# acoustic-warfare/beamforming-lk

Hardware: NVIDIA B200
Metric: power_maps_per_sec (higher is better)
Workload: dtype f32

## Files before the change

### beamforming-lk_b200/bflk/__init__.py

```python
import ctypes as C
import os

import numpy as np

_PKG = os.path.dirname(os.path.dirname(os.path.abspath(__file__)))
LIB_PATH = os.path.join(_PKG, "libbflk.so")

N_SAMPLES = 256
WINDOW = 1024
ELEMENTS = 64
SAMPLE_RATE = 48828.0
PROPAGATION_SPEED = 340.0

KERNEL_AUTO, KERNEL_GENERIC, KERNEL_TILED, KERNEL_BCAST, KERNEL_TILED_FMA2 = 0, 1, 2, 3, 4

SYMBOLS = [
    "bflk_default_config", "bflk_version", "bflk_create", "bflk_destroy", "bflk_last_error",
    "bflk_set_geometry", "bflk_set_tiled_geometry", "bflk_get_geometry", "bflk_set_channel_mask",
    "bflk_set_grid_fov", "bflk_set_grid_tables", "bflk_set_grid_shape", "bflk_set_direction_range", "bflk_get_n_directions",
    "bflk_get_grid", "bflk_get_tables", "bflk_steer_tables", "bflk_power_map", "bflk_power_map_i32",
    "bflk_power_map_batch", "bflk_power_map_batch_submit", "bflk_power_map_batch_wait", "bflk_power_map_batch_i32", "bflk_power_map_batch_i32_dev",
    "bflk_power_map_batch_dev", "bflk_power_map_batch_dev_submit", "bflk_power_map_batch_dev_join", "bflk_set_kernel", "bflk_set_channel_split", "bflk_launch_shape", "bflk_get_kernel", "bflk_launch_count", "bflk_enable_timing",
    "bflk_kernel_time_ms", "bflk_fp32_peak_tflops", "bflk_set_window", "bflk_set_window_dev", "bflk_miso", "bflk_miso_dev", "bflk_monopulse", "bflk_set_fir",
    "bflk_pin_host", "bflk_unpin_host", "bflk_heatmap", "bflk_resize_u8", "bflk_targets", "bflk_calibrate", "bflk_ingest_i32",
    "bflk_stream_open", "bflk_stream_close", "bflk_stream_push", "bflk_stream_push_i32", "bflk_stream_power_maps",
    "bflk_stream_discard", "bflk_stream_status", "bflk_stream_window",
    "bflk_comm_unique_id", "bflk_comm_init_rank", "bflk_comm_info", "bflk_shard_plan",
    "bflk_power_map_batch_sharded_dev", "bflk_power_map_batch_sharded_dev_submit", "bflk_power_map_batch_sharded_dev_join", "bflk_power_map_batch_sharded", "bflk_power_map_batch_sharded_submit", "bflk_power_map_batch_sharded_wait",
    "bflk_group_create", "bflk_group_destroy", "bflk_group_size", "bflk_group_handle", "bflk_group_last_error",
    "bflk_group_set_geometry", "bflk_group_set_tiled_geometry", "bflk_group_set_channel_mask", "bflk_group_set_grid_fov",
    "bflk_group_set_kernel", "bflk_group_power_map_batch", "bflk_group_power_map_batch_dev", "bflk_group_synchronize",
]


class Config(C.Structure):
    _fields_ = [("n_channels", C.c_int32), ("frame_len", C.c_int32), ("history", C.c_int32),
                ("window_len", C.c_int32), ("sample_rate", C.c_double), ("propagation_speed", C.c_double),
                ("device", C.c_int32), ("reserved", C.c_int32)]


class Target(C.Structure):
    _fields_ = [("theta", C.c_double), ("phi", C.c_double), ("power", C.c_float), ("probability", C.c_float),
                ("direction", C.c_int32), ("row", C.c_int32), ("col", C.c_int32), ("reserved", C.c_int32)]


# ... 27 lines not shown
    L.bflk_get_geometry.argtypes = [vp, vp]
    L.bflk_set_channel_mask.argtypes = [vp, vp, i32]
    L.bflk_set_grid_fov.argtypes = [vp, i32, i32, f32]
    L.bflk_set_grid_tables.argtypes = [vp, vp, vp, i32]
    L.bflk_set_grid_shape.argtypes = [vp, i32, i32]
    L.bflk_set_direction_range.argtypes = [vp, i32, i32]
    L.bflk_get_n_directions.argtypes = [vp, C.POINTER(i32), C.POINTER(i32), C.POINTER(i32)]
    L.bflk_get_grid.argtypes = [vp, vp, vp]
    L.bflk_get_tables.argtypes = [vp, vp, vp]
    L.bflk_steer_tables.argtypes = [vp, vp, vp, i32, vp, vp]
    L.bflk_power_map.argtypes = [vp, vp, vp]
    L.bflk_power_map_i32.argtypes = [vp, vp, vp]
    L.bflk_power_map_batch.argtypes = [vp, vp, i64, i32, vp]
    L.bflk_power_map_batch_submit.argtypes = [vp, vp, i64, i32, vp]
    L.bflk_power_map_batch_wait.argtypes = [vp]
    L.bflk_power_map_batch_i32.argtypes = [vp, vp, i64, i32, vp]
    L.bflk_power_map_batch_i32_dev.argtypes = [vp, vp, i64, i32, vp, vp]
    L.bflk_power_map_batch_dev.argtypes = [vp, vp, i64, i32, vp, vp]
    L.bflk_power_map_batch_dev_submit.argtypes = [vp, vp, i64, i32, vp, vp]
    L.bflk_power_map_batch_dev_join.argtypes = [vp, vp]
    L.bflk_set_kernel.argtypes = [vp, i32]
    L.bflk_set_channel_split.argtypes = [vp, i32]
    L.bflk_launch_shape.argtypes = [i32, i32, i32, i32, i32, i32, i32, C.POINTER(i32), C.POINTER(i32)]
    L.bflk_launch_count.argtypes = [vp]
    L.bflk_launch_count.restype = i64
    L.bflk_get_kernel.argtypes = [vp, C.POINTER(i32), C.POINTER(i32), C.POINTER(i32)]
    L.bflk_enable_timing.argtypes = [vp, i32]
    L.bflk_kernel_time_ms.argtypes = [vp, C.POINTER(f32), C.POINTER(i32), C.POINTER(f32), C.POINTER(i32)]
    L.bflk_fp32_peak_tflops.argtypes = [vp, C.POINTER(f32)]
    L.bflk_set_window.argtypes = [vp, vp]
    L.bflk_set_window_dev.argtypes = [vp, vp]
    L.bflk_miso.argtypes = [vp, vp, vp, i32, vp, vp, vp]
    L.bflk_miso_dev.argtypes = [vp, vp, vp, i32, vp, vp, vp, vp]
    L.bflk_monopulse.argtypes = [vp, vp, vp, i32, C.c_double, C.c_double, C.c_double, vp, vp, vp, vp, vp, vp]
    L.bflk_set_fir.argtypes = [vp, vp, i32, i32]
    L.bflk_heatmap.argtypes = [vp, vp, i32, vp, C.POINTER(i32), C.POINTER(f32)]
    L.bflk_pin_host.argtypes = [vp, C.c_size_t]
    L.bflk_unpin_host.argtypes = [vp]
    L.bflk_resize_u8.argtypes = [vp, vp, i32, i32, i32, i32, vp]
    L.bflk_targets.argtypes = [vp, vp, i32, f32, vp, C.POINTER(i32)]
    L.bflk_calibrate.argtypes = [vp, vp, i32, f32, vp, vp, C.POINTER(i32), C.POINTER(f32), C.POINTER(f32)]
    L.bflk_ingest_i32.argtypes = [vp, vp, i32, i32, vp]
    L.bflk_stream_open.argtypes = [vp, i32]
    L.bflk_stream_close.argtypes = [vp]
    L.bflk_stream_push.argtypes = [vp, vp, i32]
    L.bflk_stream_push_i32.argtypes = [vp, vp, i32]
# ... 37 lines not shown

def _ptr(a):
    return a.ctypes.data_as(C.c_void_p)


def shard_plan(n_directions, n_frames, n_ranks, rank, dir_groups=0):
    L = load_library()
    a, b, c, d = C.c_int32(), C.c_int32(), C.c_int32(), C.c_int32()
    rc = L.bflk_shard_plan(n_directions, n_frames, n_ranks, dir_groups, rank, C.byref(a), C.byref(b), C.byref(c), C.byref(d))
    if rc != 0:
        raise BflkError(rc, f"bflk_shard_plan({n_directions}, {n_frames}, {n_ranks}, {dir_groups}, {rank})")
    return a.value, b.value, c.value, d.value


def launch_shape(rows, cols, n_channels, n_frames=1, frame_len=256, n_sms=148, channel_split=False):
    L = load_library()
    w, s = C.c_int32(), C.c_int32()
    rc = L.bflk_launch_shape(rows, cols, n_channels, frame_len, n_frames, n_sms, 1 if channel_split else 0, C.byref(w), C.byref(s))
    if rc != 0:
        raise BflkError(rc, f"bflk_launch_shape({rows}, {cols}, {n_channels}, {frame_len}, {n_frames}, {n_sms})")
    return w.value, s.value


def comm_unique_id():
    L = load_library()
    buf = (C.c_uint8 * 128)()
    rc = L.bflk_comm_unique_id(buf)
    if rc != 0:
        raise BflkError(rc, "bflk_comm_unique_id: NCCL is not available")
    return bytes(buf)


def tile_origins(nx, ny, pitch=0.16):
    o = [[(i - (nx - 1) / 2) * pitch, (j - (ny - 1) / 2) * pitch, 0.0] for j in range(ny) for i in range(nx)]
    return np.asarray(o, np.float32)


class Beamformer:

    def __init__(self, n_channels=ELEMENTS, frame_len=N_SAMPLES, history=N_SAMPLES, window_len=WINDOW,
                 sample_rate=SAMPLE_RATE, propagation_speed=PROPAGATION_SPEED, device=0):
        self._L = load_library()
        cfg = Config()
        self._L.bflk_default_config(C.byref(cfg))
        cfg.n_channels, cfg.frame_len, cfg.history, cfg.window_len = n_channels, frame_len, history, window_len
        cfg.sample_rate, cfg.propagation_speed, cfg.device = sample_rate, propagation_speed, device
# ... 405 lines not shown
```

### beamforming-lk_b200/csrc/bflk_api.cu

```cuda
#include <algorithm>
#include <cmath>
#include <cstdlib>
#include <cstring>
#include <functional>
#include <memory>

#include "bflk_internal.h"

using namespace bflk;

static thread_local std::string g_create_error;

static int create_fail(int code, const std::string &msg) {
    g_create_error = msg;
    return code;
}

bflk_handle::~bflk_handle() {
    for (const Stream *s : {&stream, &copy_stream, &lane[0], &lane[1]}) s->sync();
    comm_release(this);
}

extern "C" {

// ... 26 lines not shown
    if (e != cudaSuccess || n_dev <= 0)
        return create_fail(BFLK_ERR_NO_DEVICE, std::string("bflk_create: no CUDA device (") + cudaGetErrorString(e) +
                                                   "); this library has no CPU fallback");
    if (cfg->device < 0 || cfg->device >= n_dev) return create_fail(BFLK_ERR_INVALID, "bflk_create: device ordinal out of range");
    cudaDeviceProp prop;
    if ((e = cudaGetDeviceProperties(&prop, cfg->device)) != cudaSuccess)
        return create_fail(BFLK_ERR_CUDA, std::string("cudaGetDeviceProperties: ") + cudaGetErrorString(e));
    if (prop.major != 10)
        return create_fail(BFLK_ERR_NO_DEVICE, "bflk_create: device is not sm_100 (kernels are built for sm_100a only)");
    if ((e = cudaSetDevice(cfg->device)) != cudaSuccess)
        return create_fail(BFLK_ERR_CUDA, std::string("cudaSetDevice: ") + cudaGetErrorString(e));
    cudaGetLastError();
    std::unique_ptr<bflk_handle> h(new bflk_handle());
    if ((e = cudaGetLastError()) != cudaSuccess)
        return create_fail(BFLK_ERR_CUDA, std::string("bflk_create: cannot create the streams and events: ") + cudaGetErrorString(e));
    h->cfg = *cfg;
    h->sm_count = prop.multiProcessorCount;
    auto env_int = [](const char *name, int dflt) { const char *v = getenv(name); return v && *v ? atoi(v) : dflt; };
    h->tuning.tile_nch = env_int("BFLK_TILE_NCH", 0);
    h->tuning.tile_warps = env_int("BFLK_TILE_WARPS", 0);
    h->tuning.tile_stages = env_int("BFLK_TILE_STAGES", 0);
    h->tuning.tile_pairs = env_int("BFLK_TILE_PAIRS", 0);
    h->tuning.tile_mode = env_int("BFLK_TILE_MODE", -1);
    h->tuning.no_ksplit = env_int("BFLK_NO_KSPLIT", 0);
    h->tuning.lat_warps = env_int("BFLK_LAT_WARPS", 0);
    h->tuning.lat_split = env_int("BFLK_LAT_SPLIT", 0);
    h->tuning.chunk_mib = env_int("BFLK_CHUNK_MIB", 0);
    *out = h.release();
    return BFLK_OK;
}

int bflk_destroy(bflk_handle *h) {
    if (!h) return BFLK_ERR_INVALID;
    cudaSetDevice(h->cfg.device);
    delete h;
    return BFLK_OK;
}

static void invalidate_tables(bflk_handle *h) {
    h->have_grid = false;
    h->tiles_valid = false;
    h->bcast_valid = false;
    h->n_dir = 0;
    h->dir_first = h->dir_count = 0;
    h->last_map_on_device = false;
}

int bflk_set_geometry(bflk_handle *h, const float *xyz, int32_t n_channels) {
    if (!h) return BFLK_ERR_INVALID;
    if (!xyz || n_channels != h->cfg.n_channels)
        return h->fail(BFLK_ERR_INVALID, "bflk_set_geometry: expected %d channels, got %d", h->cfg.n_channels, n_channels);
    BFLK_CUDA(h, cudaSetDevice(h->cfg.device));
    h->xyz.assign(xyz, xyz + 3 * (size_t)n_channels);
    BFLK_CUDA(h, h->d_xyz.reserve(3 * (size_t)n_channels));
    BFLK_CUDA(h, cudaMemcpyAsync(h->d_xyz.p, h->xyz.data(), h->xyz.size() * sizeof(float), cudaMemcpyHostToDevice, h->stream));
    BFLK_CUDA(h, cudaStreamSynchronize(h->stream));
    h->have_geometry = true;
    invalidate_tables(h);
    if (h->index.empty()) return bflk_set_channel_mask(h, nullptr, 0);
    return BFLK_OK;
}

int bflk_set_tiled_geometry(bflk_handle *h, int32_t n_tiles, const float *origins) {
    if (!h) return BFLK_ERR_INVALID;
// ... 22 lines not shown
    return BFLK_OK;
}

int bflk_set_channel_mask(bflk_handle *h, const int32_t *index, int32_t usable) {
    if (!h) return BFLK_ERR_INVALID;
    const int C = h->cfg.n_channels;
    std::vector<int32_t> idx;
    if (!index) {
        idx.resize(C);
        for (int c = 0; c < C; c++) idx[c] = c;
    } else {
        if (usable <= 0 || usable > C) return h->fail(BFLK_ERR_INVALID, "bflk_set_channel_mask: usable=%d out of range", usable);
        idx.assign(index, index + usable);
        for (int v : idx)
            if (v < 0 || v >= C) return h->fail(BFLK_ERR_INVALID, "bflk_set_channel_mask: channel %d out of range", v);
    }
    BFLK_CUDA(h, cudaSetDevice(h->cfg.device));
    h->index = idx;
    h->bcast_valid = false;
    BFLK_CUDA(h, h->d_index.reserve(idx.size()));
    BFLK_CUDA(h, cudaMemcpyAsync(h->d_index.p, h->index.data(), idx.size() * sizeof(int32_t), cudaMemcpyHostToDevice, h->stream));
    BFLK_CUDA(h, cudaStreamSynchronize(h->stream));
    h->tiles_valid = false;
    return BFLK_OK;
}

static DirTrig make_trig(double theta, double phi) {
    const float az = static_cast<float>(phi);
    const float ay = -static_cast<float>(theta);
    DirTrig t;
    t.cz = static_cast<float>(std::cos((double)az));
    t.sz = static_cast<float>(std::sin((double)az));
    t.cy = static_cast<float>(std::cos((double)ay));
    t.sy = static_cast<float>(std::sin((double)ay));
    return t;
}

static float delay_scale(const bflk_handle *h) { return (float)(h->cfg.sample_rate / h->cfg.propagation_speed); }

static int run_steer_tables(bflk_handle *h, const double *theta, const double *phi, int n, int32_t *d_off, float *d_frac,
                            int32_t *max_delay) {
    BFLK_CUDA(h, h->p_trig.reserve(n));
    BFLK_CUDA(h, h->d_trig.reserve(n));
    BFLK_CUDA(h, h->d_misc.reserve(4));
    BFLK_CUDA(h, h->p_misc.reserve(4));
    for (int i = 0; i < n; i++) h->p_trig.p[i] = make_trig(theta[i], phi[i]);
// ... 86 lines not shown
    if (min_off < 0 || max_off > h->cfg.history)
        return h->fail(BFLK_ERR_RANGE, "bflk_set_grid_tables: offsets must lie in [0, history = %d]; got [%d, %d]",
                       h->cfg.history, min_off, max_off);
    const int max_delay = h->cfg.history - min_off;
    h->theta.clear();
    h->phi.clear();
    h->rows = h->cols = 0;
    h->n_dir = n_directions;
    h->dir_first = 0;
    h->dir_count = n_directions;
    h->max_delay = max_delay;
    h->have_grid = true;
    return BFLK_OK;
}

int bflk_set_grid_shape(bflk_handle *h, int32_t rows, int32_t cols) {
    if (!h) return BFLK_ERR_INVALID;
    if (!h->have_grid) return h->fail(BFLK_ERR_STATE, "bflk_set_grid_shape: set the tables first");
    if (rows <= 0 || cols <= 0 || (int64_t)rows * cols != h->n_dir)
        return h->fail(BFLK_ERR_INVALID, "bflk_set_grid_shape: %d x %d is not the %d directions of the tables", rows, cols, h->n_dir);
    h->rows = rows;
    h->cols = cols;
    h->tiles_valid = false;
    h->bcast_valid = false;
    return BFLK_OK;
}

int bflk_set_direction_range(bflk_handle *h, int32_t first, int32_t count) {
    if (!h) return BFLK_ERR_INVALID;
    if (!h->have_grid) return h->fail(BFLK_ERR_STATE, "bflk_set_direction_range: set the grid first");
    if (first < 0 || count <= 0 || first + count > h->n_dir)
        return h->fail(BFLK_ERR_INVALID, "bflk_set_direction_range: [%d, %d) outside grid of %d", first, first + count, h->n_dir);
    h->dir_first = first;
    h->dir_count = count;
    h->tiles_valid = false;
    h->bcast_valid = false;
    h->last_map_on_device = false;
    return BFLK_OK;
}

int bflk_get_n_directions(const bflk_handle *h, int32_t *total, int32_t *first, int32_t *count) {
    if (!h || !h->have_grid) return BFLK_ERR_STATE;
    if (total) *total = h->n_dir;
    if (first) *first = h->dir_first;
    if (count) *count = h->dir_count;
    return BFLK_OK;
}

int bflk_get_grid(const bflk_handle *h, double *theta, double *phi) {
    if (!h || !h->have_grid || h->theta.empty()) return BFLK_ERR_STATE;
    if (theta) std::memcpy(theta, h->theta.data(), h->theta.size() * sizeof(double));
    if (phi) std::memcpy(phi, h->phi.data(), h->phi.size() * sizeof(double));
    return BFLK_OK;
}

int bflk_get_tables(const bflk_handle *hc, int32_t *offsets, float *fractions) {
    bflk_handle *h = const_cast<bflk_handle *>(hc);
    if (!h) return BFLK_ERR_INVALID;
// ... 121 lines not shown
    if (pack_launches) *pack_launches = n[1];
    return BFLK_OK;
}

}

namespace bflk {

int64_t min_stream_samples(const bflk_handle *h, int n_frames) {
    return (int64_t)(n_frames - 1) * h->cfg.frame_len + h->cfg.history + h->cfg.frame_len + 1;
}

int ensure_tiles(bflk_handle *h, int fast, int want_warps) {
    if (h->tiles_valid && h->tiles_fast == fast && h->tiles_want_warps == want_warps) return BFLK_OK;
    BFLK_CUDA(h, cudaEventSynchronize(h->caller_event));
    h->tiles_valid = false;
    h->tiles_fast = fast;
    h->tiles_want_warps = want_warps;
    h->tiles_usable = false;
    if (h->rows <= 0 || h->cols <= 0) {
        h->tiles_valid = true;
        return BFLK_OK;
    }
    const int cols = h->cols;
    const int row0 = (h->dir_first / cols) & ~1;
    const int row1 = (h->dir_first + h->dir_count - 1) / cols;
    const int tile_rows = (row1 - row0) / 2 + 1, tile_cols = (cols + 1) / 2;
    const int n_tiles = tile_rows * tile_cols;
    const int usable = (int)h->index.size();
    BFLK_CUDA(h, h->d_tile_dirs.reserve((size_t)n_tiles * 4));
    BFLK_CUDA(h, h->d_misc.reserve(4));
    BFLK_CUDA(h, h->p_misc.reserve(4));
    const int stage_off = das_tile_geometry(h->cfg.history, h->max_delay, 0).stage_off;
    BFLK_CUDA(h, cudaMemsetAsync(h->d_misc.p, 0, 4 * sizeof(int32_t), h->stream));
    for (int mode = 0; mode < 3; mode++) {
        BFLK_CUDA(h, launch_build_tiles(h->d_off.p, h->d_frac.p, h->cfg.n_channels, h->d_index.p, usable, h->rows, cols,
                                        h->dir_first, h->dir_count, stage_off, 0, 1, mode, -1, 0, nullptr, nullptr, n_tiles,
                                        h->d_misc.p, h->stream));
        h->launches++;
    }
    BFLK_CUDA(h, cudaMemcpyAsync(h->p_misc.p, h->d_misc.p, 3 * sizeof(int32_t), cudaMemcpyDeviceToHost, h->stream));
    BFLK_CUDA(h, cudaStreamSynchronize(h->stream));
    const int span0 = h->p_misc.p[0], span1 = h->p_misc.p[1], span2 = h->p_misc.p[2];
    int mode = 0;
    const int pair_span = std::min(span1, span2), pair_mode = span1 <= span2 ? 1 : 2;
    if (span0 > 3 && pair_span <= 3) mode = pair_mode;
    else if (span0 > 7 && pair_span <= 5) mode = pair_mode;
    const int forced = h->tuning.tile_mode;
    if (forced == 0 || ((forced == 1 || forced == 2) && h->p_misc.p[forced] <= 5)) mode = forced;
    h->n_tiles = n_tiles;
    h->tile_smax = h->p_misc.p[mode];
    h->tile_geom = das_tile_geometry(h->cfg.history, h->max_delay, h->tile_smax, n_tiles, mode, fast, &h->tuning, want_warps);
    h->tiles_usable = h->tile_smax <= das_tile_max_span() && h->cfg.frame_len >= 256 && h->cfg.frame_len % 2 == 0 &&
                      h->tile_geom.stages >= 3;
    if (!h->tiles_usable) {
        h->tiles_valid = true;
        return BFLK_OK;
    }
    const size_t entries = tile_table_entries(n_tiles, usable, h->tile_geom.warps);
    const size_t ent_bytes = das_tile_entry_bytes(h->tile_geom);
    BFLK_CUDA(h, h->d_tiles.reserve(entries * ent_bytes));
    BFLK_CUDA(h, cudaMemsetAsync(h->d_tiles.p, 0, entries * ent_bytes, h->stream));
    BFLK_CUDA(h, launch_build_tiles(h->d_off.p, h->d_frac.p, h->cfg.n_channels, h->d_index.p, usable, h->rows, cols,
                                    h->dir_first, h->dir_count, stage_off, h->tile_geom.copy_bytes, h->tile_geom.warps, mode,
                                    2 * h->tile_geom.nch - 9, fast, h->d_tiles.p,
                                    h->d_tile_dirs.p, n_tiles, h->d_misc.p, h->stream));
    h->launches++;
    BFLK_CUDA(h, cudaStreamSynchronize(h->stream));
    h->tiles_valid = true;
    return BFLK_OK;
}

}

extern "C" {

static int ensure_bcast(bflk_handle *h) {
    if (h->bcast_valid) return BFLK_OK;
    BFLK_CUDA(h, cudaEventSynchronize(h->caller_event));
    const int first = h->dir_first, count = h->dir_count;
    std::vector<int32_t> globals;
    if (h->rows > 0 && h->cols > 0) {
        float minx = 1e30f, maxx = -1e30f, miny = 1e30f, maxy = -1e30f;
        for (size_t c = 0; c < h->xyz.size() / 3; c++) {
            minx = std::min(minx, h->xyz[3 * c]); maxx = std::max(maxx, h->xyz[3 * c]);
            miny = std::min(miny, h->xyz[3 * c + 1]); maxy = std::max(maxy, h->xyz[3 * c + 1]);
        }
        const int TR = (maxx - minx >= maxy - miny) ? 8 : 4, TC = 32 / TR;
// ... 1093 lines not shown
```

### beamforming-lk_b200/csrc/bflk_internal.h

```cpp
#pragma once

#include <cuda_runtime.h>

#include <cstdarg>
#include <algorithm>
#include <cstdint>
#include <cstdio>
#include <memory>
#include <string>
#include <vector>

#include "../../include/bflk.h"

namespace bflk {

struct DirTrig {
    float cz, sz;
    float cy, sy;
};

struct __align__(16) TileEntry {
    uint32_t win_off;
    uint32_t deltas;
    int32_t span;
// ... 10 lines not shown
    float comp[4];
};

struct __align__(16) TileEntryFastDual {
    uint32_t cls_a[4], cls_b[4];
    float frac[4], comp[4];
    uint32_t deltas;
    int32_t span;
    int32_t reserved[2];
};

constexpr int kTileCC = 8;
inline size_t tile_table_entries(int n_tiles, int usable, int warps) {
    const size_t groups = (n_tiles + warps - 1) / warps, stages = (usable + kTileCC - 1) / kTileCC;
    return groups * stages * warps * kTileCC;
}

struct Tuning {
    int tile_nch = 0;
    int tile_warps = 0;
    int tile_stages = 0;
    int tile_pairs = 0;
    int tile_mode = -1;
    int lat_warps = 0;
    int lat_split = 0;
    int no_ksplit = 0;
    int chunk_mib = 0;
};

struct TileGeometry {
    int stage_off = 0;
    int nch = 0;
    int warps = 0;
    int tmpl_warps = 0;
    int fast = 0;
    int mode = 0;
    int row_chunks = 0;
    int copy_bytes = 0;
    int row_bytes = 0;
    int stages = 0;
    int pairs_per_cta = 0;
    int ksplit = 1;
};

constexpr int kBcastCC = 8;
struct BcastEntry {
// ... 93 lines not shown
    bool have_geometry = false;
    std::vector<float> xyz;
    std::vector<int32_t> index;
    bflk::DevBuf<float> d_xyz;
    bflk::DevBuf<int32_t> d_index;

    bool have_grid = false;
    int32_t rows = 0, cols = 0;
    int32_t n_dir = 0;
    int32_t dir_first = 0, dir_count = 0;
    int32_t max_delay = 0;
    std::vector<double> theta, phi;
    bflk::DevBuf<int32_t> d_off;
    bflk::DevBuf<float> d_frac;

    bool tiles_valid = false;
    bool tiles_usable = false;
    int tiles_fast = 0;
    int tiles_want_warps = 0;
    int32_t n_tiles = 0;
    int32_t tile_smax = 0;
    bflk::DevBuf<char> d_tiles;
    bflk::DevBuf<int32_t> d_tile_dirs;
    bflk::TileGeometry tile_geom;

    bool bcast_valid = false;
    int32_t bcast_tiles = 0;
    bflk::BcastGeometry bcast_geom;
    bflk::DevBuf<bflk::BcastEntry> d_bcast_table;
    bflk::DevBuf<int32_t> d_bcast_dirs;
    bflk::DevBuf<int32_t> d_bcast_globals;

    bflk::DevBuf<float> d_fir;
    int32_t fir_phases = 0, fir_taps = 0;

    const float *resident_window = nullptr;
    int64_t resident_stride = 0;
    std::unique_ptr<bflk::Session> session;
    bflk::DevBuf<int32_t> d_wire;
    bflk::DevBuf<uint8_t> d_bytes;
    bflk::DevBuf<float> d_async_in[2], d_async_out[2];
    bflk::Event async_done[2];
    uint64_t async_seq = 0;
    int async_pending = 0;
    bflk::DevBuf<float> d_maps;
    bool last_map_on_device = false;
// ... 40 lines not shown
        char buf[512];
        va_list ap;
        va_start(ap, fmt);
        vsnprintf(buf, sizeof(buf), fmt, ap);
        va_end(ap);
        error = buf;
        return code;
    }
};

#define BFLK_CUDA(h, expr)                                                                              \
    do {                                                                                                \
        cudaError_t _e = (expr);                                                                        \
        if (_e != cudaSuccess)                                                                          \
            return (h)->fail(BFLK_ERR_CUDA, "%s failed: %s (%s:%d)", #expr, cudaGetErrorString(_e), __FILE__, __LINE__); \
    } while (0)

namespace bflk {

cudaError_t launch_steer_tables(const DirTrig *d_trig, int n_dir, const float *d_xyz, int C, float k_scale,
                                int history, int32_t *d_off, float *d_frac, int32_t *d_maxdelay, cudaStream_t st);
cudaError_t launch_offset_range(const int32_t *d_off, size_t n, int32_t *d_maxoff, int32_t *d_minoff, cudaStream_t st);
cudaError_t launch_build_tiles(const int32_t *d_off, const float *d_frac, int C, const int32_t *d_index, int usable,
                               int rows, int cols, int first, int count, int stage_off, int copy_bytes, int warps,
                               int mode, int pair_span, int fast, void *d_tiles, int32_t *d_tile_dirs, int n_tiles,
                               int32_t *d_maxspan, cudaStream_t st);

struct GenericArgs {
    const float *stream;
    int64_t row_stride;
    int n_frames;
    int frame_len;
    int frame_stride;
    const int32_t *off;
    const float *frac;
    int C;
    const int32_t *index;
    int usable;
    int n_dir;
    float *power;
    float *audio;
    float norm;
    const float *fir = nullptr;
    int fir_phases = 0, fir_taps = 0;
};
cudaError_t launch_das_generic(const GenericArgs &a, cudaStream_t st);

constexpr int kMisoInline = 128;
struct MisoArgs {
// ... 114 lines not shown
```

### beamforming-lk_b200/csrc/tables.cu

```cuda
#include "bflk_internal.h"
#include "steer.cuh"

namespace bflk {

__global__ void __launch_bounds__(128) steer_tables_kernel(const DirTrig *__restrict__ trig, const float *__restrict__ xyz,
                                                           int C, float k_scale, int history, int32_t *__restrict__ off,
                                                           float *__restrict__ frac, int32_t *__restrict__ maxdelay) {
    extern __shared__ float s_del[];
    __shared__ float s_red[4];
    const int d = blockIdx.x;
    const DirTrig t = trig[d];
    float mn = INFINITY;
    for (int c = threadIdx.x; c < C; c += blockDim.x) {
        float z = steer_z(t, xyz[3 * c + 0], xyz[3 * c + 1], xyz[3 * c + 2]);
        float del = __fmul_rn(z, k_scale);
        s_del[c] = del;
        mn = fminf(mn, del);
    }
    for (int o = 16; o > 0; o >>= 1) mn = fminf(mn, __shfl_xor_sync(0xffffffffu, mn, o));
    if ((threadIdx.x & 31) == 0) s_red[threadIdx.x >> 5] = mn;
    __syncthreads();
    mn = fminf(fminf(s_red[0], s_red[1]), fminf(s_red[2], s_red[3]));
    int local_max = 0;
    for (int c = threadIdx.x; c < C; c += blockDim.x) {
// ... 22 lines not shown
        int o = off[i];
        mx = max(mx, o);
        mo = min(mo, o);
    }
    for (int o = 16; o > 0; o >>= 1) {
        mx = max(mx, __shfl_xor_sync(0xffffffffu, mx, o));
        mo = min(mo, __shfl_xor_sync(0xffffffffu, mo, o));
    }
    if ((threadIdx.x & 31) == 0) {
        atomicMax(maxoff, mx);
        atomicMin(minoff, mo);
    }
}

cudaError_t launch_offset_range(const int32_t *d_off, size_t n, int32_t *d_maxoff, int32_t *d_minoff, cudaStream_t st) {
    int blocks = (int)((n + 255) / 256);
    if (blocks > 1184) blocks = 1184;
    if (blocks < 1) blocks = 1;
    max_delay_kernel<<<blocks, 256, 0, st>>>(d_off, n, d_maxoff, d_minoff);
    return cudaGetLastError();
}

__global__ void build_tiles_kernel(const int32_t *__restrict__ off, const float *__restrict__ frac, int C,
                                   const int32_t *__restrict__ index, int usable, int rows, int cols, int first,
                                   int count, int stage_off, int copy_bytes, int warps, int mode, int pair_span,
                                   int fast, void *__restrict__ tiles_raw,
                                   int32_t *__restrict__ tile_dirs, int n_tiles, int tile_cols, int row0,
                                   int32_t *__restrict__ maxspan) {
    const int t = blockIdx.x;
    if (t >= n_tiles) return;
    TileEntry *tiles = fast ? nullptr : static_cast<TileEntry *>(tiles_raw);
    TileEntryFast *tiles_fast = fast && mode == 0 ? static_cast<TileEntryFast *>(tiles_raw) : nullptr;
    TileEntryFastDual *tiles_fast2 = fast && mode != 0 ? static_cast<TileEntryFastDual *>(tiles_raw) : nullptr;
    const int tr = t / tile_cols, tc = t % tile_cols;
    int dirs[4];
#pragma unroll
    for (int slot = 0; slot < 4; slot++) {
        const int q = mode == 1 ? ((slot & 1) << 1 | (slot >> 1)) : slot;
        int r = row0 + 2 * tr + (q >> 1), c = 2 * tc + (q & 1);
        dirs[slot] = (r < rows && c < cols) ? r * cols + c : -1;
    }
    int ref = dirs[0];
#pragma unroll
    for (int slot = 1; slot < 4; slot++)
        if (ref < 0) ref = dirs[slot];
    if (threadIdx.x < 4 && tile_dirs) {
        int g = dirs[threadIdx.x];
        tile_dirs[4 * t + threadIdx.x] = (g >= first && g < first + count) ? g - first : -1;
    }
    int span_max = 0;
    for (int s = threadIdx.x; s < usable; s += blockDim.x) {
        const int c = index[s];
        int o[4];
        TileEntry e;
#pragma unroll
        for (int slot = 0; slot < 4; slot++) {
            int g = dirs[slot] >= 0 ? dirs[slot] : ref;
            o[slot] = off[(size_t)g * C + c];
            e.frac[slot] = frac[(size_t)g * C + c];
        }
        unsigned packed = 0, need_last = 0;
        int span = 0;
        if (mode == 0) {
            const int base = min(min(o[0], o[1]), min(o[2], o[3]));
// ... 57 lines not shown
            for (int w = 0; w < 2; w++) {
                const unsigned wo = (e.win_off >> (16 * w)) & 0xffffu, r = (packed >> (24 + 2 * w)) & 3;
#pragma unroll
                for (int k = 0; k < 4; k++)
                    (w ? q.cls_b : q.cls_a)[k] = (unsigned)(s % kTileCC) * 2u * (unsigned)copy_bytes + wo + ((k > 0 && r >= (unsigned)(4 - k)) ? 16u : 0u);
            }
            q.deltas = (packed & 0x10ffffffu) | need_last;
            q.span = span;
            q.reserved[0] = q.reserved[1] = 0;
#pragma unroll
            for (int k = 0; k < 4; k++) {
                q.frac[k] = e.frac[k];
                q.comp[k] = __fsub_rn(1.0f, e.frac[k]);
            }
            tiles_fast2[slot] = q;
        }
        span_max = max(span_max, span);
    }
    for (int o = 16; o > 0; o >>= 1) span_max = max(span_max, __shfl_xor_sync(0xffffffffu, span_max, o));
    if ((threadIdx.x & 31) == 0) atomicMax(maxspan + mode, span_max);
}

cudaError_t launch_build_tiles(const int32_t *d_off, const float *d_frac, int C, const int32_t *d_index, int usable,
                               int rows, int cols, int first, int count, int stage_off, int copy_bytes, int warps,
                               int mode, int pair_span, int fast, void *d_tiles, int32_t *d_tile_dirs, int n_tiles,
                               int32_t *d_maxspan, cudaStream_t st) {
    const int row0 = (first / cols) & ~1;
    const int tile_cols = (cols + 1) / 2;
    build_tiles_kernel<<<n_tiles, 128, 0, st>>>(d_off, d_frac, C, d_index, usable, rows, cols, first, count, stage_off,
                                                copy_bytes, warps, mode, pair_span, fast, d_tiles, d_tile_dirs, n_tiles, tile_cols, row0, d_maxspan);
    return cudaGetLastError();
}

}
```

### include/bflk.h

```cpp
#ifndef BFLK_H
#define BFLK_H

#include <stddef.h>
#include <stdint.h>

#ifdef __cplusplus
extern "C" {
#endif

#define BFLK_VERSION 1

typedef enum bflk_status {
    BFLK_OK = 0,
    BFLK_ERR_INVALID = -1,
    BFLK_ERR_STATE = -2,
    BFLK_ERR_CUDA = -3,
    BFLK_ERR_NO_DEVICE = -4,
    BFLK_ERR_RANGE = -5
} bflk_status;

typedef struct bflk_config {
    int32_t n_channels;
    int32_t frame_len;
    int32_t history;
// ... 25 lines not shown
int bflk_get_n_directions(const bflk_handle *h, int32_t *total, int32_t *first, int32_t *count);
int bflk_get_grid(const bflk_handle *h, double *theta, double *phi);
int bflk_get_tables(const bflk_handle *h, int32_t *offsets, float *fractions);
int bflk_steer_tables(bflk_handle *h, const double *theta, const double *phi, int32_t n_targets,
                      int32_t *offsets, float *fractions);

int bflk_power_map(bflk_handle *h, const float *window, float *power_out);
int bflk_power_map_batch(bflk_handle *h, const float *stream, int64_t n_samples, int32_t n_frames, float *power_out);
int bflk_power_map_batch_submit(bflk_handle *h, const float *stream, int64_t n_samples, int32_t n_frames, float *power_out);
int bflk_power_map_batch_wait(bflk_handle *h);
int bflk_power_map_i32(bflk_handle *h, const int32_t *frames, float *power_out);
int bflk_power_map_batch_i32(bflk_handle *h, const int32_t *frames, int64_t n_samples, int32_t n_frames, float *power_out);
int bflk_power_map_batch_i32_dev(bflk_handle *h, const int32_t *frames_dev, int64_t n_samples, int32_t n_frames,
                                 float *power_dev, void *cuda_stream);
int bflk_power_map_batch_dev(bflk_handle *h, const float *stream_dev, int64_t n_samples, int32_t n_frames,
                             float *power_dev, void *cuda_stream);
int bflk_power_map_batch_dev_submit(bflk_handle *h, const float *stream_dev, int64_t n_samples, int32_t n_frames,
                                    float *power_dev, void *cuda_stream);
int bflk_power_map_batch_dev_join(bflk_handle *h, void *cuda_stream);
int bflk_set_kernel(bflk_handle *h, int32_t which);
int bflk_set_channel_split(bflk_handle *h, int32_t on);
int bflk_launch_shape(int32_t rows, int32_t cols, int32_t n_channels, int32_t frame_len, int32_t n_frames, int32_t n_sms,
                      int32_t channel_split, int32_t *warps, int32_t *split);
int bflk_get_kernel(const bflk_handle *h, int32_t *last_used, int32_t *tile_span, int32_t *window_chunks);
int64_t bflk_launch_count(const bflk_handle *h);
int bflk_enable_timing(bflk_handle *h, int32_t on);
int bflk_fp32_peak_tflops(bflk_handle *h, float *tflops);
int bflk_kernel_time_ms(bflk_handle *h, float *das_ms, int32_t *das_launches, float *pack_ms, int32_t *pack_launches);

int bflk_stream_open(bflk_handle *h, int32_t max_frames);
int bflk_stream_close(bflk_handle *h);
int bflk_stream_push(bflk_handle *h, const float *samples, int32_t n);
int bflk_stream_push_i32(bflk_handle *h, const int32_t *rows, int32_t n);
int bflk_stream_power_maps(bflk_handle *h, int32_t max_frames, float *power_out, int64_t *first_frame, int32_t *n_frames);
int bflk_stream_discard(bflk_handle *h, int32_t keep);
int bflk_stream_status(const bflk_handle *h, int64_t *pushed, int64_t *next_frame, int32_t *ready, int64_t *skipped);
int bflk_stream_window(bflk_handle *h, int64_t frame);

int bflk_comm_unique_id(uint8_t *id128);
int bflk_comm_init_rank(bflk_handle *h, const uint8_t *id128, int32_t n_ranks, int32_t rank, int32_t dir_groups);
int bflk_comm_info(const bflk_handle *h, int32_t *n_ranks, int32_t *rank, int32_t *dir_groups, int32_t *frame_groups,
                   int64_t *collectives);
int bflk_shard_plan(int32_t n_directions, int32_t n_frames, int32_t n_ranks, int32_t dir_groups, int32_t rank,
                    int32_t *dir_first, int32_t *dir_count, int32_t *frame_first, int32_t *frame_count);
int bflk_power_map_batch_sharded_dev(bflk_handle *h, const float *stream_dev, int64_t n_samples, int32_t n_frames,
                                     float *power_all_dev, void *cuda_stream);
// ... 58 lines not shown
```

Measured before the change: 77730.

## Group tiled-kernel directions by delay similarity via matching instead of fixed 2x2 grid

Replaces the fixed 2x2 grid assignment of directions to tiles with a host-side grouping. The grouping pairs directions by delay-offset similarity using greedy-plus-augmenting matching, then pairs those pairs into tiles and refines them with local swaps. Tiles are sorted by window cost and passed to the tile builder as an explicit direction list. The aim is to cut the number of channels whose delay spread exceeds the shared window, lowering per-tile sample loads in the dual (mode != 0) tiled kernel. The grouping adds host-side setup cost, and a new error path triggers if a grouped pair's spread exceeds the window.

```diff
diff --git a/beamforming-lk_b200/bflk/__init__.py b/beamforming-lk_b200/bflk/__init__.py
--- a/beamforming-lk_b200/bflk/__init__.py
+++ b/beamforming-lk_b200/bflk/__init__.py
@@ -20,7 +20,7 @@
     "bflk_set_grid_fov", "bflk_set_grid_tables", "bflk_set_grid_shape", "bflk_set_direction_range", "bflk_get_n_directions",
     "bflk_get_grid", "bflk_get_tables", "bflk_steer_tables", "bflk_power_map", "bflk_power_map_i32",
     "bflk_power_map_batch", "bflk_power_map_batch_submit", "bflk_power_map_batch_wait", "bflk_power_map_batch_i32", "bflk_power_map_batch_i32_dev",
-    "bflk_power_map_batch_dev", "bflk_power_map_batch_dev_submit", "bflk_power_map_batch_dev_join", "bflk_set_kernel", "bflk_set_channel_split", "bflk_launch_shape", "bflk_get_kernel", "bflk_launch_count", "bflk_enable_timing",
+    "bflk_power_map_batch_dev", "bflk_power_map_batch_dev_submit", "bflk_power_map_batch_dev_join", "bflk_set_kernel", "bflk_set_channel_split", "bflk_launch_shape", "bflk_tile_grouping", "bflk_get_kernel", "bflk_launch_count", "bflk_enable_timing",
     "bflk_kernel_time_ms", "bflk_fp32_peak_tflops", "bflk_set_window", "bflk_set_window_dev", "bflk_miso", "bflk_miso_dev", "bflk_monopulse", "bflk_set_fir",
     "bflk_pin_host", "bflk_unpin_host", "bflk_heatmap", "bflk_resize_u8", "bflk_targets", "bflk_calibrate", "bflk_ingest_i32",
     "bflk_stream_open", "bflk_stream_close", "bflk_stream_push", "bflk_stream_push_i32", "bflk_stream_power_maps",
@@ -94,6 +94,7 @@
     L.bflk_set_kernel.argtypes = [vp, i32]
     L.bflk_set_channel_split.argtypes = [vp, i32]
     L.bflk_launch_shape.argtypes = [i32, i32, i32, i32, i32, i32, i32, C.POINTER(i32), C.POINTER(i32)]
+    L.bflk_tile_grouping.argtypes = [vp, i32, i32, i32, i32, i32, vp, C.POINTER(i32), C.POINTER(i64)]
     L.bflk_launch_count.argtypes = [vp]
     L.bflk_launch_count.restype = i64
     L.bflk_get_kernel.argtypes = [vp, C.POINTER(i32), C.POINTER(i32), C.POINTER(i32)]
@@ -177,6 +178,17 @@
     return w.value, s.value
 
 
+def tile_grouping(offsets, cols, first, pair_span):
+    L = load_library()
+    off = _np(offsets, np.int32)
+    tiles = np.empty((off.shape[0], 4), np.int32)
+    n, wb = C.c_int32(), C.c_int64()
+    rc = L.bflk_tile_grouping(_ptr(off), off.shape[0], off.shape[1], cols, first, pair_span, _ptr(tiles), C.byref(n), C.byref(wb))
+    if rc != 0:
+        raise BflkError(rc, f"bflk_tile_grouping({off.shape}, {cols}, {first}, {pair_span})")
+    return tiles[:n.value].copy(), wb.value
+
+
 def comm_unique_id():
     L = load_library()
     buf = (C.c_uint8 * 128)()
diff --git a/beamforming-lk_b200/csrc/bflk_api.cu b/beamforming-lk_b200/csrc/bflk_api.cu
--- a/beamforming-lk_b200/csrc/bflk_api.cu
+++ b/beamforming-lk_b200/csrc/bflk_api.cu
@@ -72,6 +72,7 @@
     h->tuning.tile_stages = env_int("BFLK_TILE_STAGES", 0);
     h->tuning.tile_pairs = env_int("BFLK_TILE_PAIRS", 0);
     h->tuning.tile_mode = env_int("BFLK_TILE_MODE", -1);
+    h->tuning.tile_group = env_int("BFLK_TILE_GROUP", 1);
     h->tuning.no_ksplit = env_int("BFLK_NO_KSPLIT", 0);
     h->tuning.lat_warps = env_int("BFLK_LAT_WARPS", 0);
     h->tuning.lat_split = env_int("BFLK_LAT_SPLIT", 0);
@@ -90,6 +91,7 @@
 static void invalidate_tables(bflk_handle *h) {
     h->have_grid = false;
     h->tiles_valid = false;
+    h->tile_groups.clear();
     h->bcast_valid = false;
     h->n_dir = 0;
     h->dir_first = h->dir_count = 0;
@@ -158,6 +160,7 @@
     BFLK_CUDA(h, cudaMemcpyAsync(h->d_index.p, h->index.data(), idx.size() * sizeof(int32_t), cudaMemcpyHostToDevice, h->stream));
     BFLK_CUDA(h, cudaStreamSynchronize(h->stream));
     h->tiles_valid = false;
+    h->tile_groups.clear();
     return BFLK_OK;
 }
 
@@ -290,6 +293,7 @@
     h->rows = rows;
     h->cols = cols;
     h->tiles_valid = false;
+    h->tile_groups.clear();
     h->bcast_valid = false;
     return BFLK_OK;
 }
@@ -302,6 +306,7 @@
     h->dir_first = first;
     h->dir_count = count;
     h->tiles_valid = false;
+    h->tile_groups.clear();
     h->bcast_valid = false;
     h->last_map_on_device = false;
     return BFLK_OK;
@@ -469,21 +474,22 @@
         h->tiles_valid = true;
         return BFLK_OK;
     }
-    const int cols = h->cols;
-    const int row0 = (h->dir_first / cols) & ~1;
-    const int row1 = (h->dir_first + h->dir_count - 1) / cols;
-    const int tile_rows = (row1 - row0) / 2 + 1, tile_cols = (cols + 1) / 2;
-    const int n_tiles = tile_rows * tile_cols;
+    const int C = h->cfg.n_channels, first = h->dir_first, count = h->dir_count;
     const int usable = (int)h->index.size();
-    BFLK_CUDA(h, h->d_tile_dirs.reserve((size_t)n_tiles * 4));
     BFLK_CUDA(h, h->d_misc.reserve(4));
     BFLK_CUDA(h, h->p_misc.reserve(4));
     const int stage_off = das_tile_geometry(h->cfg.history, h->max_delay, 0).stage_off;
+    std::vector<int32_t> grid[3];
+    for (int mode = 0; mode < 3; mode++) grid[mode] = grid_tiles(h->rows, h->cols, first, count, mode);
+    int n_tiles = (int)(grid[0].size() / 4);
+    BFLK_CUDA(h, h->d_tile_list.reserve(3 * grid[0].size()));
+    for (int mode = 0; mode < 3; mode++)
+        BFLK_CUDA(h, cudaMemcpyAsync(h->d_tile_list.p + mode * grid[0].size(), grid[mode].data(), grid[0].size() * sizeof(int32_t),
+                                     cudaMemcpyHostToDevice, h->stream));
     BFLK_CUDA(h, cudaMemsetAsync(h->d_misc.p, 0, 4 * sizeof(int32_t), h->stream));
     for (int mode = 0; mode < 3; mode++) {
-        BFLK_CUDA(h, launch_build_tiles(h->d_off.p, h->d_frac.p, h->cfg.n_channels, h->d_index.p, usable, h->rows, cols,
-                                        h->dir_first, h->dir_count, stage_off, 0, 1, mode, -1, 0, nullptr, nullptr, n_tiles,
-                                        h->d_misc.p, h->stream));
+        BFLK_CUDA(h, launch_build_tiles(h->d_off.p, h->d_frac.p, C, h->d_index.p, usable, h->d_tile_list.p + mode * grid[0].size(),
+                                        first, count, stage_off, 0, 1, mode, -1, 0, nullptr, nullptr, n_tiles, h->d_misc.p, h->stream));
         h->launches++;
     }
     BFLK_CUDA(h, cudaMemcpyAsync(h->p_misc.p, h->d_misc.p, 3 * sizeof(int32_t), cudaMemcpyDeviceToHost, h->stream));
@@ -504,13 +510,44 @@
         h->tiles_valid = true;
         return BFLK_OK;
     }
+    const int32_t *d_list = h->d_tile_list.p + mode * grid[0].size();
+    if (mode != 0 && h->tuning.tile_group != 0) {
+        const int pair_span = 2 * h->tile_geom.nch - 9;
+        if (h->tile_groups.empty() || h->tile_groups_span != pair_span) {
+            std::vector<int32_t> rows((size_t)count * C), off((size_t)count * usable);
+            BFLK_CUDA(h, cudaMemcpyAsync(rows.data(), h->d_off.p + (size_t)first * C, rows.size() * sizeof(int32_t),
+                                         cudaMemcpyDeviceToHost, h->stream));
+            BFLK_CUDA(h, cudaStreamSynchronize(h->stream));
+            for (int d = 0; d < count; d++)
+                for (int s = 0; s < usable; s++) off[(size_t)d * usable + s] = rows[(size_t)d * C + h->index[s]];
+            h->tile_groups = group_tiles(off.data(), count, usable, h->cols, first, pair_span).dirs;
+            h->tile_groups_span = pair_span;
+        }
+        n_tiles = (int)(h->tile_groups.size() / 4);
+        BFLK_CUDA(h, h->d_tile_list.reserve(h->tile_groups.size()));
+        BFLK_CUDA(h, cudaMemcpyAsync(h->d_tile_list.p, h->tile_groups.data(), h->tile_groups.size() * sizeof(int32_t),
+                                     cudaMemcpyHostToDevice, h->stream));
+        d_list = h->d_tile_list.p;
+        BFLK_CUDA(h, cudaMemsetAsync(h->d_misc.p + mode, 0, sizeof(int32_t), h->stream));
+        BFLK_CUDA(h, launch_build_tiles(h->d_off.p, h->d_frac.p, C, h->d_index.p, usable, d_list, first, count, stage_off, 0, 1,
+                                        mode, -1, 0, nullptr, nullptr, n_tiles, h->d_misc.p, h->stream));
+        h->launches++;
+        BFLK_CUDA(h, cudaMemcpyAsync(h->p_misc.p, h->d_misc.p, 3 * sizeof(int32_t), cudaMemcpyDeviceToHost, h->stream));
+        BFLK_CUDA(h, cudaStreamSynchronize(h->stream));
+        if (h->p_misc.p[mode] > pair_span)
+            return h->fail(BFLK_ERR_STATE, "ensure_tiles: a grouped direction pair spreads over %d samples, its window serves %d",
+                           h->p_misc.p[mode], pair_span);
+        h->n_tiles = n_tiles;
+        h->tile_smax = h->p_misc.p[mode];
+        h->tile_geom = das_tile_geometry(h->cfg.history, h->max_delay, h->tile_smax, n_tiles, mode, fast, &h->tuning, want_warps);
+    }
+    BFLK_CUDA(h, h->d_tile_dirs.reserve((size_t)n_tiles * 4));
     const size_t entries = tile_table_entries(n_tiles, usable, h->tile_geom.warps);
     const size_t ent_bytes = das_tile_entry_bytes(h->tile_geom);
     BFLK_CUDA(h, h->d_tiles.reserve(entries * ent_bytes));
     BFLK_CUDA(h, cudaMemsetAsync(h->d_tiles.p, 0, entries * ent_bytes, h->stream));
-    BFLK_CUDA(h, launch_build_tiles(h->d_off.p, h->d_frac.p, h->cfg.n_channels, h->d_index.p, usable, h->rows, cols,
-                                    h->dir_first, h->dir_count, stage_off, h->tile_geom.copy_bytes, h->tile_geom.warps, mode,
-                                    2 * h->tile_geom.nch - 9, fast, h->d_tiles.p,
+    BFLK_CUDA(h, launch_build_tiles(h->d_off.p, h->d_frac.p, C, h->d_index.p, usable, d_list, first, count, stage_off,
+                                    h->tile_geom.copy_bytes, h->tile_geom.warps, mode, 2 * h->tile_geom.nch - 9, fast, h->d_tiles.p,
                                     h->d_tile_dirs.p, n_tiles, h->d_misc.p, h->stream));
     h->launches++;
     BFLK_CUDA(h, cudaStreamSynchronize(h->stream));
diff --git a/beamforming-lk_b200/csrc/bflk_internal.h b/beamforming-lk_b200/csrc/bflk_internal.h
--- a/beamforming-lk_b200/csrc/bflk_internal.h
+++ b/beamforming-lk_b200/csrc/bflk_internal.h
@@ -56,6 +56,7 @@
     int tile_stages = 0;
     int tile_pairs = 0;
     int tile_mode = -1;
+    int tile_group = 1;
     int lat_warps = 0;
     int lat_split = 0;
     int no_ksplit = 0;
@@ -195,6 +196,9 @@
     int32_t tile_smax = 0;
     bflk::DevBuf<char> d_tiles;
     bflk::DevBuf<int32_t> d_tile_dirs;
+    bflk::DevBuf<int32_t> d_tile_list;
+    std::vector<int32_t> tile_groups;
+    int tile_groups_span = 0;
     bflk::TileGeometry tile_geom;
 
     bool bcast_valid = false;
@@ -281,9 +285,16 @@
                                 int history, int32_t *d_off, float *d_frac, int32_t *d_maxdelay, cudaStream_t st);
 cudaError_t launch_offset_range(const int32_t *d_off, size_t n, int32_t *d_maxoff, int32_t *d_minoff, cudaStream_t st);
 cudaError_t launch_build_tiles(const int32_t *d_off, const float *d_frac, int C, const int32_t *d_index, int usable,
-                               int rows, int cols, int first, int count, int stage_off, int copy_bytes, int warps,
+                               const int32_t *d_list, int first, int count, int stage_off, int copy_bytes, int warps,
                                int mode, int pair_span, int fast, void *d_tiles, int32_t *d_tile_dirs, int n_tiles,
                                int32_t *d_maxspan, cudaStream_t st);
+std::vector<int32_t> grid_tiles(int rows, int cols, int first, int count, int mode);
+
+struct TileGrouping {
+    std::vector<int32_t> dirs;
+    int64_t window_b = 0;
+};
+TileGrouping group_tiles(const int32_t *off, int count, int usable, int cols, int first, int pair_span);
 
 struct GenericArgs {
     const float *stream;
diff --git a/beamforming-lk_b200/csrc/tables.cu b/beamforming-lk_b200/csrc/tables.cu
--- a/beamforming-lk_b200/csrc/tables.cu
+++ b/beamforming-lk_b200/csrc/tables.cu
@@ -68,24 +68,18 @@
 }
 
 __global__ void build_tiles_kernel(const int32_t *__restrict__ off, const float *__restrict__ frac, int C,
-                                   const int32_t *__restrict__ index, int usable, int rows, int cols, int first,
-                                   int count, int stage_off, int copy_bytes, int warps, int mode, int pair_span,
+                                   const int32_t *__restrict__ index, int usable, const int32_t *__restrict__ list,
+                                   int first, int count, int stage_off, int copy_bytes, int warps, int mode, int pair_span,
                                    int fast, void *__restrict__ tiles_raw,
-                                   int32_t *__restrict__ tile_dirs, int n_tiles, int tile_cols, int row0,
-                                   int32_t *__restrict__ maxspan) {
+                                   int32_t *__restrict__ tile_dirs, int n_tiles, int32_t *__restrict__ maxspan) {
     const int t = blockIdx.x;
     if (t >= n_tiles) return;
     TileEntry *tiles = fast ? nullptr : static_cast<TileEntry *>(tiles_raw);
     TileEntryFast *tiles_fast = fast && mode == 0 ? static_cast<TileEntryFast *>(tiles_raw) : nullptr;
     TileEntryFastDual *tiles_fast2 = fast && mode != 0 ? static_cast<TileEntryFastDual *>(tiles_raw) : nullptr;
-    const int tr = t / tile_cols, tc = t % tile_cols;
     int dirs[4];
 #pragma unroll
-    for (int slot = 0; slot < 4; slot++) {
-        const int q = mode == 1 ? ((slot & 1) << 1 | (slot >> 1)) : slot;
-        int r = row0 + 2 * tr + (q >> 1), c = 2 * tc + (q & 1);
-        dirs[slot] = (r < rows && c < cols) ? r * cols + c : -1;
-    }
+    for (int slot = 0; slot < 4; slot++) dirs[slot] = list[4 * t + slot];
     int ref = dirs[0];
 #pragma unroll
     for (int slot = 1; slot < 4; slot++)
@@ -189,14 +183,25 @@
 }
 
 cudaError_t launch_build_tiles(const int32_t *d_off, const float *d_frac, int C, const int32_t *d_index, int usable,
-                               int rows, int cols, int first, int count, int stage_off, int copy_bytes, int warps,
+                               const int32_t *d_list, int first, int count, int stage_off, int copy_bytes, int warps,
                                int mode, int pair_span, int fast, void *d_tiles, int32_t *d_tile_dirs, int n_tiles,
                                int32_t *d_maxspan, cudaStream_t st) {
-    const int row0 = (first / cols) & ~1;
-    const int tile_cols = (cols + 1) / 2;
-    build_tiles_kernel<<<n_tiles, 128, 0, st>>>(d_off, d_frac, C, d_index, usable, rows, cols, first, count, stage_off,
-                                                copy_bytes, warps, mode, pair_span, fast, d_tiles, d_tile_dirs, n_tiles, tile_cols, row0, d_maxspan);
+    build_tiles_kernel<<<n_tiles, 128, 0, st>>>(d_off, d_frac, C, d_index, usable, d_list, first, count, stage_off,
+                                                copy_bytes, warps, mode, pair_span, fast, d_tiles, d_tile_dirs, n_tiles, d_maxspan);
     return cudaGetLastError();
 }
 
-}
+std::vector<int32_t> grid_tiles(int rows, int cols, int first, int count, int mode) {
+    const int row0 = (first / cols) & ~1, row1 = (first + count - 1) / cols;
+    const int tile_rows = (row1 - row0) / 2 + 1, tile_cols = (cols + 1) / 2;
+    std::vector<int32_t> list((size_t)tile_rows * tile_cols * 4);
+    for (int t = 0; t < tile_rows * tile_cols; t++)
+        for (int slot = 0; slot < 4; slot++) {
+            const int q = mode == 1 ? ((slot & 1) << 1 | (slot >> 1)) : slot;
+            const int r = row0 + 2 * (t / tile_cols) + (q >> 1), c = 2 * (t % tile_cols) + (q & 1);
+            list[4 * t + slot] = (r < rows && c < cols) ? r * cols + c : -1;
+        }
+    return list;
+}
+
+}
diff --git a/beamforming-lk_b200/csrc/tile_group.cu b/beamforming-lk_b200/csrc/tile_group.cu
--- /dev/null
+++ b/beamforming-lk_b200/csrc/tile_group.cu
@@ -0,0 +1,195 @@
+#include <algorithm>
+#include <cstdint>
+#include <vector>
+#include <cstdlib>
+
+#include "bflk_internal.h"
+
+namespace bflk {
+
+namespace {
+
+constexpr int kRadius = 3;
+constexpr int kRounds = 4;
+
+struct Edge {
+    int64_t w;
+    int a, b;
+    bool operator<(const Edge &o) const { return w != o.w ? w < o.w : (a != o.a ? a < o.a : b < o.b); }
+};
+
+std::vector<int> match(int n, std::vector<Edge> &edges) {
+    std::sort(edges.begin(), edges.end());
+    std::vector<int> mate(n, -1);
+    std::vector<std::vector<int>> adj(n);
+    for (const Edge &e : edges) {
+        adj[e.a].push_back(e.b);
+        adj[e.b].push_back(e.a);
+        if (mate[e.a] < 0 && mate[e.b] < 0) { mate[e.a] = e.b; mate[e.b] = e.a; }
+    }
+    std::vector<int> parent(n), seen(n, -1), queue;
+    for (int u = 0; u < n; u++) {
+        if (mate[u] >= 0 || adj[u].empty()) continue;
+        queue.assign(1, u);
+        seen[u] = u;
+        int end = -1, end_from = -1;
+        for (size_t qi = 0; qi < queue.size() && end < 0; qi++) {
+            const int y = queue[qi];
+            for (int x : adj[y]) {
+                if (seen[x] == u || x == mate[y]) continue;
+                if (mate[x] < 0) { end = x; end_from = y; break; }
+                seen[x] = u;
+                if (seen[mate[x]] == u) continue;
+                seen[mate[x]] = u;
+                parent[mate[x]] = x;
+                parent[x] = y;
+                queue.push_back(mate[x]);
+            }
+        }
+        if (end < 0) continue;
+        int x = end, y = end_from;
+        while (true) {
+            const int next = mate[y];
+            mate[y] = x;
+            mate[x] = y;
+            if (y == u) break;
+            x = next;
+            y = parent[x];
+        }
+    }
+    return mate;
+}
+
+}
+
+TileGrouping group_tiles(const int32_t *off, int count, int usable, int cols, int first, int pair_span) {
+    TileGrouping out;
+    if (count <= 0 || usable <= 0 || cols <= 0) return out;
+    auto row = [&](int d) { return off + (size_t)d * usable; };
+    auto pos_r = [&](int d) { return (first + d) / cols; };
+    auto pos_c = [&](int d) { return (first + d) % cols; };
+    auto local_at = [&](int r, int c) -> int {
+        if (r < 0 || c < 0 || c >= cols) return -1;
+        const int64_t g = (int64_t)r * cols + c - first;
+        return g >= 0 && g < count ? (int)g : -1;
+    };
+
+    std::vector<Edge> edges;
+    for (int a = 0; a < count; a++)
+        for (int dr = -kRadius; dr <= kRadius; dr++)
+            for (int dc = -kRadius; dc <= kRadius; dc++) {
+                const int b = local_at(pos_r(a) + dr, pos_c(a) + dc);
+                if (b <= a) continue;
+                const int32_t *oa = row(a), *ob = row(b);
+                int64_t w = 0;
+                int mx = 0;
+                for (int s = 0; s < usable && mx <= pair_span; s++) {
+                    const int d = std::abs(oa[s] - ob[s]);
+                    w += d;
+                    mx = std::max(mx, d);
+                }
+                if (mx <= pair_span) edges.push_back({w, a, b});
+            }
+    std::vector<int> mate = match(count, edges);
+    std::vector<int> pa, pb, pair_of(count, -1);
+    for (int a = 0; a < count; a++) {
+        if (mate[a] >= 0 && mate[a] < a) continue;
+        pair_of[a] = (int)pa.size();
+        if (mate[a] >= 0) pair_of[mate[a]] = (int)pa.size();
+        pa.push_back(a);
+        pb.push_back(mate[a]);
+    }
+    const int np = (int)pa.size();
+    std::vector<int32_t> lo((size_t)np * usable), hi((size_t)np * usable);
+    for (int p = 0; p < np; p++)
+        for (int s = 0; s < usable; s++) {
+            const int32_t x = row(pa[p])[s], y = pb[p] >= 0 ? row(pb[p])[s] : x;
+            lo[(size_t)p * usable + s] = std::min(x, y);
+            hi[(size_t)p * usable + s] = std::max(x, y);
+        }
+    auto cost = [&](int p, int q) {
+        const int32_t *lp = &lo[(size_t)p * usable], *hp = &hi[(size_t)p * usable];
+        if (q < 0) return 0;
+        const int32_t *lq = &lo[(size_t)q * usable], *hq = &hi[(size_t)q * usable];
+        int n = 0;
+        for (int s = 0; s < usable; s++) n += std::max(hp[s], hq[s]) - std::min(lp[s], lq[s]) > pair_span;
+        return n;
+    };
+    std::vector<int> stamp(np, -1);
+    auto neighbours = [&](int p, std::vector<int> &nb) {
+        nb.clear();
+        stamp[p] = p;
+        for (int dr = -kRadius; dr <= kRadius; dr++)
+            for (int dc = -kRadius; dc <= kRadius; dc++) {
+                const int x = local_at(pos_r(pa[p]) + dr, pos_c(pa[p]) + dc);
+                if (x < 0 || stamp[pair_of[x]] == p) continue;
+                stamp[pair_of[x]] = p;
+                nb.push_back(pair_of[x]);
+            }
+        std::sort(nb.begin(), nb.end());
+    };
+
+    std::vector<Edge> pedges;
+    std::vector<int> nb;
+    for (int p = 0; p < np; p++) {
+        neighbours(p, nb);
+        for (int q : nb)
+            if (q > p && (pb[p] >= 0 || pb[q] >= 0)) pedges.push_back({cost(p, q), p, q});
+    }
+    std::vector<int> tmate = match(np, pedges);
+    auto ok = [&](int p, int q) { return q < 0 || pb[p] >= 0 || pb[q] >= 0; };
+    for (int round = 0; round < kRounds; round++) {
+        bool changed = false;
+        for (int p = 0; p < np; p++) {
+            neighbours(p, nb);
+            for (int q : nb) {
+                const int p2 = tmate[p], q2 = tmate[q];
+                if (q == p2 || p2 < 0 || q2 < 0) continue;
+                const int now = cost(p, p2) + cost(q, q2);
+                if (now == 0) continue;
+                const int alt1 = ok(p, q) && ok(p2, q2) ? cost(p, q) + cost(p2, q2) : now;
+                const int alt2 = ok(p, q2) && ok(p2, q) ? cost(p, q2) + cost(p2, q) : now;
+                if (alt1 < now && alt1 <= alt2) {
+                    tmate[p] = q; tmate[q] = p; tmate[p2] = q2; tmate[q2] = p2;
+                    changed = true;
+                } else if (alt2 < now) {
+                    tmate[p] = q2; tmate[q2] = p; tmate[p2] = q; tmate[q] = p2;
+                    changed = true;
+                }
+            }
+        }
+        if (!changed) break;
+    }
+
+    struct Tile { int d[4]; int cost; };
+    std::vector<Tile> tiles;
+    for (int p = 0; p < np; p++) {
+        int q = tmate[p], p0 = p;
+        if (q >= 0 && q < p) continue;
+        if (q >= 0 && pb[q] < 0) std::swap(p0, q);
+        tiles.push_back({{pa[p0], pb[p0], q >= 0 ? pa[q] : -1, q >= 0 ? pb[q] : -1}, cost(p0, q)});
+    }
+
+    static const int exp_order = [] { const char *e = getenv("BFLK_EXP_ORDER"); return e ? atoi(e) : 0; }();
+    if (exp_order == 0) std::stable_sort(tiles.begin(), tiles.end(), [](const Tile &x, const Tile &y) { return x.cost > y.cost; });
+    if (exp_order == 2) std::stable_sort(tiles.begin(), tiles.end(), [](const Tile &x, const Tile &y) { return x.cost < y.cost; });
+    out.dirs.reserve(4 * tiles.size());
+    for (const Tile &t : tiles) {
+        for (int k = 0; k < 4; k++) out.dirs.push_back(t.d[k] >= 0 ? first + t.d[k] : -1);
+        out.window_b += t.cost;
+    }
+    return out;
+}
+
+}
+
+extern "C" int bflk_tile_grouping(const int32_t *offsets, int32_t n_directions, int32_t n_channels, int32_t cols,
+                                  int32_t first, int32_t pair_span, int32_t *tiles, int32_t *n_tiles, int64_t *window_b) {
+    if (!offsets || !tiles || !n_tiles || n_directions <= 0 || n_channels <= 0 || cols <= 0 || first < 0 || pair_span < 0)
+        return BFLK_ERR_INVALID;
+    const bflk::TileGrouping g = bflk::group_tiles(offsets, n_directions, n_channels, cols, first, pair_span);
+    std::copy(g.dirs.begin(), g.dirs.end(), tiles);
+    *n_tiles = (int32_t)(g.dirs.size() / 4);
+    if (window_b) *window_b = g.window_b;
+    return BFLK_OK;
+}
diff --git a/include/bflk.h b/include/bflk.h
--- a/include/bflk.h
+++ b/include/bflk.h
@@ -71,6 +71,8 @@
 int bflk_set_channel_split(bflk_handle *h, int32_t on);
 int bflk_launch_shape(int32_t rows, int32_t cols, int32_t n_channels, int32_t frame_len, int32_t n_frames, int32_t n_sms,
                       int32_t channel_split, int32_t *warps, int32_t *split);
+int bflk_tile_grouping(const int32_t *offsets, int32_t n_directions, int32_t n_channels, int32_t cols, int32_t first,
+                       int32_t pair_span, int32_t *tiles, int32_t *n_tiles, int64_t *window_b);
 int bflk_get_kernel(const bflk_handle *h, int32_t *last_used, int32_t *tile_span, int32_t *window_chunks);
 int64_t bflk_launch_count(const bflk_handle *h);
 int bflk_enable_timing(bflk_handle *h, int32_t on);
```

New measurement: 80040 (median of 6 runs). +3.0%, better.
